# carry4985/ORB_SLAM2_MAP

Hardware: AMD Instinct MI355X
Metric: frames/sec ORB extract+match (640x480, 1000 feat) (higher is better)
Workload: dtype u8; 1 GPU; C2: synthetic 640x480 RGB-D stream, 1000 features, 8 levels, extract + BF-Hamming match of consecutive frames; resident_frame_pool=1024, sequences=1, parallelism=1 sequence per GPU, schedule_name=best, extraction_parts=1

## Files before the change

### include/orbgpu.h

```cpp
#ifndef ORBGPU_H
#define ORBGPU_H

#include <stddef.h>
#include <stdint.h>

#ifdef __cplusplus
extern "C" {
#endif

#define ORBGPU_ABI_VERSION 1
#define ORBGPU_MAX_LEVELS 16

typedef enum {
    ORBGPU_OK = 0,
    ORBGPU_EINVAL = -1,
    ORBGPU_ENOMEM = -2,
    ORBGPU_EHIP = -3,
    ORBGPU_ECAPACITY = -4,
    ORBGPU_ELEVEL = -5
} orbgpu_status;

const char *orbgpu_last_error_string(void);
int orbgpu_abi_version(void);
int orbgpu_device_count(void);
// ... 59 lines not shown
};
int orbgpu_extractor_debug_read(orbgpu_extractor *h, int32_t what, int32_t frame, int32_t level, void *dst,
                                size_t dst_bytes, size_t *n, int32_t *aux);

int orbgpu_extractor_graph_state(const orbgpu_extractor *h, int32_t *state);
int orbgpu_extractor_debug_quadtree_config(const orbgpu_extractor *h, int32_t batch, int32_t *lds_keys, int32_t *threads,
                                           int32_t *lds_bytes);
int orbgpu_extractor_set_profiling(orbgpu_extractor *h, int32_t enable);
int orbgpu_extractor_set_concurrent_blur(orbgpu_extractor *h, int32_t enable);
int orbgpu_extractor_set_fast_early_out(orbgpu_extractor *h, int32_t enable);

int orbgpu_extractor_set_stage_signal(orbgpu_extractor *h, int32_t stage, void *hip_event);
int orbgpu_extractor_stage_count(void);
const char *orbgpu_extractor_stage_name(int32_t i);
int orbgpu_extractor_stage_times(orbgpu_extractor *h, float *ms_out);

typedef struct orbgpu_pipeline orbgpu_pipeline;
int orbgpu_pipeline_create(const orbgpu_extractor_params *params, int32_t parts, orbgpu_pipeline **out);
int orbgpu_pipeline_destroy(orbgpu_pipeline *pl);
int orbgpu_pipeline_parts(const orbgpu_pipeline *pl, int32_t *parts);
int orbgpu_pipeline_part(orbgpu_pipeline *pl, int32_t k, orbgpu_extractor **part);
int orbgpu_pipeline_extract_device(orbgpu_pipeline *pl, const uint8_t *d_gray, int32_t batch, int32_t width,
                                   int32_t height, size_t stride, size_t frame_stride, orbgpu_keypoint *d_kps,
                                   uint8_t *d_desc, int32_t cap, int32_t *d_n_out, void *wait_event, void *done_event);
int orbgpu_pipeline_wait(orbgpu_pipeline *pl, void *hip_stream);


#define ORBGPU_TH_HIGH 100
#define ORBGPU_TH_LOW 50
#define ORBGPU_HISTO_LENGTH 30
#define ORBGPU_GRID_COLS 64
#define ORBGPU_GRID_ROWS 48

int orbgpu_hamming256(const uint8_t *a, const uint8_t *b, int32_t n, int32_t *out, int32_t device_id);

int orbgpu_distinctive_descriptors(int32_t groups, const int32_t *offsets, const uint8_t *desc, int32_t *best_idx,
                                   int32_t device_id);

int orbgpu_match_bf(const uint8_t *desc_a, const float *angle_a, const uint8_t *valid_a, int32_t na,
                    const uint8_t *desc_b, const float *angle_b, int32_t nb, int32_t th_low, float nnratio,
                    int32_t check_orientation, int32_t *match_b, int32_t *nmatches, int32_t device_id);

typedef struct orbgpu_matcher orbgpu_matcher;
int orbgpu_matcher_create(int32_t device_id, int32_t max_pairs, int32_t cap, orbgpu_matcher **out);
int orbgpu_matcher_destroy(orbgpu_matcher *m);
int orbgpu_match_bf_batch_device(orbgpu_matcher *m, int32_t pairs, int32_t cap, const uint8_t *d_desc_a,
                                 const void *d_angle_a, const uint8_t *d_valid_a, const int32_t *d_na,
                                 const uint8_t *d_desc_b, const void *d_angle_b, const int32_t *d_nb,
                                 size_t angle_stride_bytes, int32_t th_low, float nnratio,
                                 int32_t check_orientation, int32_t *d_match_b, int32_t *d_nmatches,
                                 void *hip_stream);
int orbgpu_matcher_last_sweeps(orbgpu_matcher *m, int32_t *sweeps);
int orbgpu_matcher_last_launch(orbgpu_matcher *m, int32_t *nsplit, int32_t *stage_b, int32_t *resolve_threads);

typedef struct {
    int32_t n;
    const float *kp_x, *kp_y;
    const int32_t *kp_octave;
    const float *kp_angle;
    const float *u_right;
    const uint8_t *desc;
    float min_x, max_x, min_y, max_y;
    float grid_inv_w, grid_inv_h;
    const float *scale_factors;
    int32_t nlevels;
    const int32_t *cell_start;
    const int32_t *cell_items;
} orbgpu_frame_view;

int orbgpu_assign_features_to_grid(int32_t n, const float *kp_x, const float *kp_y, float min_x, float min_y,
                                   float grid_inv_w, float grid_inv_h, int32_t *cell_start, int32_t *cell_items);

typedef struct orbgpu_camera {
    float fx, fy, cx, cy;
    float dist[5];
    float mbf;
    float min_x, max_x, min_y, max_y;
} orbgpu_camera;

int orbgpu_undistort_points(int32_t n, const float *xy_in, const orbgpu_camera *cam, float *xy_out, int32_t device_id);

int orbgpu_frame_glue_batch_device(int32_t device_id, int32_t batch, int32_t cap, const orbgpu_keypoint *d_kps,
                                   const int32_t *d_n, const float *d_depth, size_t depth_stride,
                                   size_t depth_frame_stride, const orbgpu_camera *cam, orbgpu_keypoint *d_kps_un,
                                   float *d_u_right, float *d_kp_depth, int32_t *d_cell_start,
                                   int32_t *d_cell_items, void *hip_stream);


int orbgpu_stereo_matches_batch_device(const orbgpu_extractor *left, int32_t left_frame0, const orbgpu_extractor *right,
                                       int32_t right_frame0, int32_t batch, int32_t cap, const orbgpu_keypoint *d_kps_l,
                                       const int32_t *d_n_l, const uint8_t *d_desc_l, const orbgpu_keypoint *d_kps_r,
                                       const int32_t *d_n_r, const uint8_t *d_desc_r, float mbf, float fx,
                                       float *d_u_right, float *d_depth, int32_t *d_n_stereo, void *hip_stream);
int orbgpu_compute_stereo_matches(const orbgpu_extractor *left, const orbgpu_extractor *right, int32_t n_l,
                                  const orbgpu_keypoint *kps_l, const uint8_t *desc_l, int32_t n_r,
                                  const orbgpu_keypoint *kps_r, const uint8_t *desc_r, float mbf, float fx,
                                  float *u_right, float *depth);

typedef struct orbgpu_device_frame_view {
    int32_t cap;
    const int32_t *n;
    const orbgpu_keypoint *kps;
    const uint8_t *desc;
    const float *u_right;
    const int32_t *cell_start;
    const int32_t *cell_items;
// ... 461 lines not shown
```

### orb_slam2_map_amd/csrc/matcher_bf.hip

```cpp
#include "common.h"
#include "matcher_common.h"
#include "staging.h"

#include <algorithm>
#include <climits>
#include <cstdlib>
#include <new>
#include <vector>

namespace orbgpu {

constexpr int BF_TOPK = 4;
constexpr uint32_t BF_KEY_NONE = 0xFFFFFFFFu;

__device__ __forceinline__ uint32_t bf_key(int dist, int j) { return ((uint32_t)dist << 12) | (uint32_t)j; }
__device__ __forceinline__ int bf_key_dist(uint32_t k) { return k == BF_KEY_NONE ? 256 : (int)(k >> 12); }
__device__ __forceinline__ int bf_key_idx(uint32_t k) { return (int)(k & 0xFFFu); }

__device__ __forceinline__ void cswap(uint32_t &a, uint32_t &b)
{
    const uint32_t lo = min(a, b), hi = max(a, b);
    a = lo;
    b = hi;
}

__device__ __forceinline__ void top4_insert(uint32_t t[4], uint32_t k)
{
    if (k < t[3]) {
        t[3] = k;
        cswap(t[2], t[3]);
        cswap(t[1], t[2]);
        cswap(t[0], t[1]);
    }
}

__device__ __forceinline__ void top4_merge(uint32_t t[4], const uint32_t o[4])
{
    uint32_t c0 = min(t[0], o[3]), c1 = min(t[1], o[2]), c2 = min(t[2], o[1]), c3 = min(t[3], o[0]);
    cswap(c0, c2);
    cswap(c1, c3);
    cswap(c0, c1);
    cswap(c2, c3);
    cswap(c1, c2);
    t[0] = c0;
    t[1] = c1;
    t[2] = c2;
    t[3] = c3;
}

constexpr int BF_MIN_SPLIT = 1, BF_MAX_SPLIT = 16;
constexpr size_t BF_RESOLVE_MAX_LDS = 150 * 1024;
constexpr int BF_TILE_STRIDE = 272;
constexpr int BF_TILE_ROWS = 64;
constexpr int BF_TOPK_THREADS = 512;
constexpr int BF_TOPK_ROWS = BF_TOPK_THREADS / 64 * 32;

typedef int v4i __attribute__((ext_vector_type(4)));
typedef int v16i __attribute__((ext_vector_type(16)));

template <uint32_t PM = 0x000001FFu> __device__ __forceinline__ v4i bf_expand16(uint32_t hw)
{
    v4i r;
#pragma unroll
    for (int q = 0; q < 4; q++) {
        const uint32_t n = (hw >> (4 * q)) & 0xFu;
        const uint32_t w01 = __umul24(n, 0x00204081u) & 0x01010101u;
        r[q] = (int)__builtin_amdgcn_perm(0u, PM, w01);
    }
    return r;
}

__device__ __forceinline__ v4i bf_expand16_01(uint32_t hw)
{
    v4i r;
#pragma unroll
    for (int q = 0; q < 4; q++)
        r[q] = (int)(__umul24((hw >> (4 * q)) & 0xFu, 0x00204081u) & 0x01010101u);
    return r;
}

template <bool NODES>
__global__ __launch_bounds__(BF_TOPK_THREADS) void k_bf_topk(int cap, const uint8_t *__restrict__ desc_a,
                                                 const int *__restrict__ na_p, const uint8_t *__restrict__ desc_b,
                                                 const int *__restrict__ nb_p, uint32_t *__restrict__ topk,
                                                 int acc_min, const int *__restrict__ node_a,
                                                 const int *__restrict__ node_b)
{
    __shared__ __align__(16) uint8_t s_tile[2][BF_TILE_ROWS * BF_TILE_STRIDE];
    const int nsplit = gridDim.z;
    const int pair = blockIdx.y;
    const int na = min(na_p[pair], cap);
    const int nb = min(nb_p[pair], cap);
    if ((int)(blockIdx.x * BF_TOPK_ROWS) >= na)
        return;
    const int tid = threadIdx.x, lane = tid & 63, wave = tid >> 6;
    const int r = lane & 31, h = lane >> 5;
    const int i = blockIdx.x * BF_TOPK_ROWS + wave * 32 + r;
    int my_node = 0;
    const int *nodes_b = nullptr;
    if (NODES) {
        my_node = node_a[(size_t)pair * cap + min(i, na - 1)];
        nodes_b = node_b + (size_t)pair * cap;
    }
    v4i fa[8];
    {
        const uint32_t *ga = reinterpret_cast<const uint32_t *>(desc_a + ((size_t)pair * cap + min(i, na - 1)) * 32);
#pragma unroll
        for (int s = 0; s < 8; s++)
            fa[s] = bf_expand16<0x000020E0u>(ga[s] >> (16 * h));
    }
    const int per = (nb + nsplit - 1) / nsplit;
    const int jbeg = (int)blockIdx.z * per, jend = min(nb, jbeg + per);
    const int ntiles = (jend - jbeg + BF_TILE_ROWS - 1) / BF_TILE_ROWS;
    const uint32_t *gb = reinterpret_cast<const uint32_t *>(desc_b + (size_t)pair * cap * 32);
    const int sm = tid >> 3, sw = tid & 7;
    auto fetch = [&](int tile) {
        const int j = min(jbeg + tile * BF_TILE_ROWS + sm, nb - 1);
        return gb[(size_t)j * 8 + sw];
    };
    auto stage = [&](uint32_t d, int buf) {
        v4i *dst = reinterpret_cast<v4i *>(&s_tile[buf][sm * BF_TILE_STRIDE + sw * 32]);
        dst[0] = bf_expand16_01(d);
        dst[1] = bf_expand16_01(d >> 16);
    };
    v16i tag;
    {
        const uint32_t *ga = reinterpret_cast<const uint32_t *>(desc_a + ((size_t)pair * cap + min(i, na - 1)) * 32);
        int pop = 0;
#pragma unroll
        for (int s = 0; s < 8; s++)
            pop += __popc(ga[s]);
        const int sa16 = 16 * (2 * pop - 256);
#pragma unroll
        for (int reg = 0; reg < 16; reg++)
            tag[reg] = (15 - reg) - sa16;
    }
    uint32_t t[4] = {BF_KEY_NONE, BF_KEY_NONE, BF_KEY_NONE, BF_KEY_NONE};
    int lim = acc_min;
    uint32_t d_next = 0;
    if (ntiles > 0)
        stage(fetch(0), 0);
    if (ntiles > 1)
        d_next = fetch(1);
    __syncthreads();
    for (int tile = 0; tile < ntiles; tile++) {
        const uint32_t d_cur = d_next;
        if (tile + 2 < ntiles)
            d_next = fetch(tile + 2);
        if (tile + 1 < ntiles)
            stage(d_cur, (tile + 1) & 1);
        const uint8_t *tb = &s_tile[tile & 1][r * BF_TILE_STRIDE + h * 16];
        v16i acc0 = tag, acc1 = tag;
#pragma unroll
        for (int s = 0; s < 8; s++) {
            const v4i fb0 = *reinterpret_cast<const v4i *>(tb + s * 32);
            const v4i fb1 = *reinterpret_cast<const v4i *>(tb + 32 * BF_TILE_STRIDE + s * 32);
            acc0 = __builtin_amdgcn_mfma_i32_32x32x32_i8(fb0, fa[s], acc0, 0, 0, 0);
            acc1 = __builtin_amdgcn_mfma_i32_32x32x32_i8(fb1, fa[s], acc1, 0, 0, 0);
        }
        const int jlast = jend - 1;
#pragma unroll
        for (int u = 0; u < 2; u++) {
            const v16i &acc = u ? acc1 : acc0;
            int e[16];
#pragma unroll
            for (int reg = 0; reg < 16; reg++)
                e[reg] = acc[reg];
            const int j0 = jbeg + tile * BF_TILE_ROWS + 32 * u + 4 * h;
            for (;;) {
                int m = max(max(e[0], e[1]), e[2]);
#pragma unroll
                for (int reg = 3; reg < 15; reg += 2)
                    m = max(max(m, e[reg]), e[reg + 1]);
                m = max(m, e[15]);
                const bool hit = (m >> 4) >= lim;
                if (!__any(hit))
                    break;
                if (hit) {
                    const int reg = 15 - (m & 15);
                    const int j = j0 + (reg & 3) + 8 * (reg >> 2);
                    if (j <= jlast && (!NODES || nodes_b[j] == my_node)) {
                        top4_insert(t, (uint32_t)(((256 - (m >> 4)) << 11) + j));
                        if (t[3] != BF_KEY_NONE)
                            lim = max(lim, 256 - 2 * (int)(t[3] >> 12));
                    }
#pragma unroll
                    for (int r2 = 0; r2 < 16; r2++)
                        e[r2] = e[r2] == m ? INT_MIN : e[r2];
                }
            }
        }
        __syncthreads();
    }
    {
        uint32_t o[4];
#pragma unroll
        for (int k = 0; k < 4; k++)
            o[k] = __shfl_xor(t[k], 32, 64);
        top4_merge(t, o);
    }
    if (h == 0 && i < na)
        *reinterpret_cast<uint4 *>(topk + (((size_t)pair * cap + i) * nsplit + blockIdx.z) * BF_TOPK) =
            make_uint4(t[0], t[1], t[2], t[3]);
}

__device__ __forceinline__ void bf_full_scan_wave(const uint64_t *__restrict__ ga, const uint64_t *gb, int i, int nb,
                                  const int *claim, int &b1, int &i1, int &b2, const int *__restrict__ nodes_b,
                                  int my_node)
{
    const int lane = threadIdx.x & 63;
    uint64_t a[4] = {ga[(size_t)i * 4], ga[(size_t)i * 4 + 1], ga[(size_t)i * 4 + 2], ga[(size_t)i * 4 + 3]};
    int v1 = 256, vi = INT_MAX, v2 = 256;
    for (int j = lane; j < nb; j += 64) {
        if (claim[j] < i)
            continue;
        if (nodes_b && nodes_b[j] != my_node)
            continue;
        uint64_t b[4] = {gb[(size_t)j * 4], gb[(size_t)j * 4 + 1], gb[(size_t)j * 4 + 2], gb[(size_t)j * 4 + 3]};
        const int d = hamming256(a, b);
        if (d < v1) {
            v2 = v1;
            v1 = d;
            vi = j;
        } else if (d < v2) {
            v2 = d;
        }
    }
#pragma unroll
    for (int off = 32; off > 0; off >>= 1) {
        const int o1 = __shfl_xor(v1, off, 64), oi = __shfl_xor(vi, off, 64), o2 = __shfl_xor(v2, off, 64);
        const bool other_first = (o1 < v1) || (o1 == v1 && oi < vi);
        const int n2 = min(min(v2, o2), max(v1, o1));
        v1 = other_first ? o1 : v1;
        vi = other_first ? oi : vi;
        v2 = n2;
    }
    b1 = v1;
    i1 = vi == INT_MAX ? -1 : vi;
    b2 = v2;
}

__device__ __forceinline__ void bf_load_keys(const uint32_t *__restrict__ tk, int i, int nsplit, uint32_t key[4])
{
    const uint4 k4 = *reinterpret_cast<const uint4 *>(tk + (size_t)i * nsplit * BF_TOPK);
    key[0] = k4.x, key[1] = k4.y, key[2] = k4.z, key[3] = k4.w;
    for (int sp = 1; sp < nsplit; sp++) {
// ... 216 lines not shown
{
    extern __shared__ __align__(16) uint8_t smem[];
    __shared__ unsigned long long s_best;
    uint64_t *sd = reinterpret_cast<uint64_t *>(smem);
    const int g = blockIdx.x, tid = threadIdx.x;
    const int beg = offsets[g], n = offsets[g + 1] - beg;
    if (n <= 0) {
        if (tid == 0)
            best_idx[g] = -1;
        return;
    }
    const uint64_t *gd = reinterpret_cast<const uint64_t *>(desc) + (size_t)beg * 4;
    for (int x = tid; x < n * 4; x += 256)
        sd[x] = gd[x];
    if (tid == 0)
        s_best = ~0ull;
    __syncthreads();
    const int k = (n - 1) >> 1;
    unsigned long long mine = ~0ull;
    for (int i = tid; i < n; i += 256) {
        const uint64_t a[4] = {sd[i * 4], sd[i * 4 + 1], sd[i * 4 + 2], sd[i * 4 + 3]};
        int lo = 0, hi = 256;
        while (lo < hi) {
            const int mid = (lo + hi) >> 1;
            int cnt = 0;
            for (int j = 0; j < n; j++) {
                const uint64_t b[4] = {sd[j * 4], sd[j * 4 + 1], sd[j * 4 + 2], sd[j * 4 + 3]};
                cnt += hamming256(a, b) <= mid ? 1 : 0;
            }
            if (cnt >= k + 1)
                hi = mid;
            else
                lo = mid + 1;
        }
        const unsigned long long key = ((unsigned long long)lo << 32) | (unsigned)i;
        mine = key < mine ? key : mine;
    }
    atomicMin(&s_best, mine);
    __syncthreads();
    if (tid == 0)
        best_idx[g] = (int)(s_best & 0xFFFFFFFFull);
}

}

using namespace orbgpu;

struct orbgpu_matcher {
    int device_id = 0;
    int max_pairs = 0, cap = 0;
    DevBuf d_topk, d_sweeps;
    int last_pairs = 0;
    int resolve_threads = 1024;
    int last_nsplit = 0, last_stage_b = 0;
};

static int matcher_destroy_impl(orbgpu_matcher *m)
{
    if (!m)
        return ORBGPU_OK;
    (void)hipSetDevice(m->device_id);
    (void)hipDeviceSynchronize();
    m->d_topk.release();
    m->d_sweeps.release();
    delete m;
    return ORBGPU_OK;
}

extern "C" {

int orbgpu_matcher_create(int32_t device_id, int32_t max_pairs, int32_t cap, orbgpu_matcher **out)
{
    std::lock_guard<std::mutex> lifecycle(orbgpu::lifecycle_mutex());
    ORBGPU_REQUIRE(out, "null argument");
    ORBGPU_REQUIRE(max_pairs >= 1 && cap >= 1 && cap <= 4096, "max_pairs must be >= 1 and cap in [1,4096]");
    int rc = select_device(device_id);
    if (rc != ORBGPU_OK)
        return rc;
    orbgpu_matcher *m = new (std::nothrow) orbgpu_matcher();
    if (!m) {
        set_error("out of host memory");
        return ORBGPU_ENOMEM;
    }
    m->device_id = device_id;
    m->max_pairs = max_pairs;
    m->cap = cap;
    if (const char *q = getenv("ORBGPU_DEBUG_BF_RESOLVE_THREADS")) {
        const int v = atoi(q);
        if (v == 256 || v == 512 || v == 1024)
            m->resolve_threads = v;
    }
    const size_t P = (size_t)max_pairs;
    if ((rc = m->d_topk.reserve(sizeof(uint32_t) * std::max<size_t>(P * BF_MIN_SPLIT, BF_MAX_SPLIT) * cap * BF_TOPK)) != ORBGPU_OK ||
        (rc = m->d_sweeps.reserve(sizeof(int) * P)) != ORBGPU_OK) {
        matcher_destroy_impl(m);
        return rc;
    }
    hipError_t he = hipFuncSetAttribute(reinterpret_cast<const void *>(k_bf_resolve),
                                 hipFuncAttributeMaxDynamicSharedMemorySize, BF_RESOLVE_MAX_LDS);
    if (he != hipSuccess) {
        set_error("hipFuncSetAttribute: %s", hipGetErrorString(he));
        matcher_destroy_impl(m);
        return ORBGPU_EHIP;
    }
    *out = m;
    return ORBGPU_OK;
}

int orbgpu_matcher_destroy(orbgpu_matcher *m)
{
    std::lock_guard<std::mutex> lifecycle(orbgpu::lifecycle_mutex());
    return matcher_destroy_impl(m);
}

static int match_batch_device(orbgpu_matcher *m, int32_t pairs, int32_t cap, const uint8_t *d_desc_a,
                              const void *d_angle_a, const uint8_t *d_valid_a, const int32_t *d_node_a, const int32_t *d_na,
                              const uint8_t *d_desc_b, const void *d_angle_b, const int32_t *d_node_b, const int32_t *d_nb,
                              size_t angle_stride, int32_t th_low, float nnratio, int32_t check_orientation,
                              int32_t *d_match_b, int32_t *d_nmatches, void *hip_stream)
{
    ORBGPU_REQUIRE(m && d_desc_a && d_desc_b && d_na && d_nb && d_match_b && d_nmatches, "null argument");
    ORBGPU_REQUIRE(pairs >= 1 && pairs <= m->max_pairs && cap >= 1 && cap <= m->cap,
                   "pairs/cap exceed the matcher's capacity (%d pairs, cap %d)", m->max_pairs, m->cap);
    ORBGPU_REQUIRE(!check_orientation || (d_angle_a && d_angle_b && angle_stride >= 4 && angle_stride % 4 == 0),
                   "orientation check needs 4-byte aligned angle arrays");
    int rc = select_device(m->device_id);
    if (rc != ORBGPU_OK)
        return rc;
    hipStream_t st = (hipStream_t)hip_stream;
    uint32_t *topk = m->d_topk.as<uint32_t>();
    int nsplit = BF_MIN_SPLIT;
    while (nsplit < BF_MAX_SPLIT && (size_t)pairs * ((cap + BF_TOPK_ROWS - 1) / BF_TOPK_ROWS) * (BF_TOPK_THREADS / 64) * nsplit < 2048 &&
           (size_t)pairs * nsplit * 2 <= std::max<size_t>((size_t)m->max_pairs * BF_MIN_SPLIT, BF_MAX_SPLIT))
        nsplit *= 2;
    const dim3 grid((cap + BF_TOPK_ROWS - 1) / BF_TOPK_ROWS, pairs, nsplit);
    int dmax = std::min(std::max(th_low, 0), 256);
    while (dmax < 256 && !(nnratio * (float)(dmax + 1) > (float)th_low))
        dmax++;
    if (d_node_a)
        hipLaunchKernelGGL(k_bf_topk<true>, grid, dim3(BF_TOPK_THREADS), 0, st, cap, d_desc_a, d_na, d_desc_b, d_nb, topk,
                           256 - 2 * dmax, d_node_a, d_node_b);
    else
        hipLaunchKernelGGL(k_bf_topk<false>, grid, dim3(BF_TOPK_THREADS), 0, st, cap, d_desc_a, d_na, d_desc_b, d_nb, topk,
                           256 - 2 * dmax, (const int *)nullptr, (const int *)nullptr);
    const int stage_b = (size_t)48 * cap <= BF_RESOLVE_MAX_LDS ? 1 : 0;
    const size_t lds = (size_t)(stage_b ? 48 : 16) * cap;
    hipLaunchKernelGGL(k_bf_resolve, dim3(pairs), dim3(m->resolve_threads), lds, st, cap, d_desc_a, d_valid_a, d_na,
                       d_desc_b, d_nb, topk, th_low, nnratio, reinterpret_cast<const uint8_t *>(d_angle_a),
                       reinterpret_cast<const uint8_t *>(d_angle_b), angle_stride, check_orientation, d_match_b,
                       d_nmatches, m->d_sweeps.as<int>(), stage_b, nsplit, d_node_a, d_node_b);
    ORBGPU_HIP_TRY(hipGetLastError());
    m->last_pairs = pairs;
    m->last_nsplit = nsplit;
    m->last_stage_b = stage_b;
    return ORBGPU_OK;
}

int orbgpu_match_bf_batch_device(orbgpu_matcher *m, int32_t pairs, int32_t cap, const uint8_t *d_desc_a,
                                 const void *d_angle_a, const uint8_t *d_valid_a, const int32_t *d_na,
                                 const uint8_t *d_desc_b, const void *d_angle_b, const int32_t *d_nb,
                                 size_t angle_stride, int32_t th_low, float nnratio, int32_t check_orientation,
                                 int32_t *d_match_b, int32_t *d_nmatches, void *hip_stream)
{
    return match_batch_device(m, pairs, cap, d_desc_a, d_angle_a, d_valid_a, nullptr, d_na, d_desc_b, d_angle_b, nullptr,
                              d_nb, angle_stride, th_low, nnratio, check_orientation, d_match_b, d_nmatches, hip_stream);
}

int orbgpu_search_by_bow_batch_device(orbgpu_matcher *m, int32_t pairs, int32_t cap, const uint8_t *d_desc_a,
                                      const void *d_angle_a, const uint8_t *d_valid_a, const int32_t *d_node_a,
                                      const int32_t *d_na, const uint8_t *d_desc_b, const void *d_angle_b,
                                      const int32_t *d_node_b, const int32_t *d_nb, size_t angle_stride, int32_t th_low,
                                      float nnratio, int32_t check_orientation, int32_t *d_match_b,
                                      int32_t *d_nmatches, void *hip_stream)
{
    ORBGPU_REQUIRE(d_node_a && d_node_b, "null node arrays");
    return match_batch_device(m, pairs, cap, d_desc_a, d_angle_a, d_valid_a, d_node_a, d_na, d_desc_b, d_angle_b, d_node_b,
                              d_nb, angle_stride, th_low, nnratio, check_orientation, d_match_b, d_nmatches, hip_stream);
}

int orbgpu_matcher_last_sweeps(orbgpu_matcher *m, int32_t *sweeps)
{
    ORBGPU_REQUIRE(m && sweeps, "null argument");
    ORBGPU_REQUIRE(m->last_pairs > 0, "no call recorded");
    int rc = select_device(m->device_id);
    if (rc != ORBGPU_OK)
        return rc;
    ORBGPU_HIP_TRY(hipDeviceSynchronize());
    ORBGPU_HIP_TRY(hipMemcpy(sweeps, m->d_sweeps.p, sizeof(int) * m->last_pairs, hipMemcpyDeviceToHost));
    return ORBGPU_OK;
}

int orbgpu_matcher_last_launch(orbgpu_matcher *m, int32_t *nsplit, int32_t *stage_b, int32_t *resolve_threads)
{
    ORBGPU_REQUIRE(m && nsplit && stage_b && resolve_threads, "null argument");
    ORBGPU_REQUIRE(m->last_pairs > 0, "no call recorded");
    *nsplit = m->last_nsplit;
    *stage_b = m->last_stage_b;
    *resolve_threads = m->resolve_threads;
    return ORBGPU_OK;
}

static int match_host(const uint8_t *desc_a, const float *angle_a, const uint8_t *valid_a, const int32_t *node_a,
                      int32_t na, const uint8_t *desc_b, const float *angle_b, const int32_t *node_b, int32_t nb,
                      int32_t th_low, float nnratio, int32_t check_orientation, int32_t *match_b, int32_t *nmatches,
                      int32_t device_id)
{
    ORBGPU_REQUIRE(match_b && nmatches, "null argument");
    ORBGPU_REQUIRE(na >= 0 && nb >= 0 && na <= 4096 && nb <= 4096, "na/nb must be in [0,4096]");
    ORBGPU_REQUIRE((na == 0 || desc_a) && (nb == 0 || desc_b), "null descriptors");
    ORBGPU_REQUIRE(!check_orientation || ((na == 0 || angle_a) && (nb == 0 || angle_b)), "null angles");
    if (na == 0 || nb == 0) {
        int rc = select_device(device_id);
        if (rc != ORBGPU_OK)
            return rc;
        for (int j = 0; j < nb; j++)
            match_b[j] = -1;
        *nmatches = 0;
        return ORBGPU_OK;
    }
    enum { DA, DB, AA, AB, VA, CNT, MB, NM, NDA, NDB, N_BUF };
    struct Ws : Staging<N_BUF> {
        int cap = 0;
        orbgpu_matcher *m = nullptr;
        void drop_matcher()
        {
            if (m)
                orbgpu_matcher_destroy(m);
            m = nullptr;
        }
        ~Ws() { release([this] { drop_matcher(); }); }
    };
    int rc = select_device(device_id);
    if (rc != ORBGPU_OK)
        return rc;
    Ws &ws = per_device_workspace<Ws>(device_id);
    if ((rc = ws.bind(device_id, true)) != ORBGPU_OK)
        return rc;
    const int need = std::max(na, nb);
    if (ws.cap < need) {
        ws.drop_matcher();
        ws.cap = 0;
// ... 153 lines not shown
```

### orb_slam2_map_amd/lib.py

```python
import ctypes as C
import os
import sys

import numpy as np

HERE = os.path.dirname(os.path.abspath(__file__))
LIB_PATH = os.path.join(HERE, "liborbgpu.so")

OK, EINVAL, ENOMEM, EHIP, ECAPACITY, ELEVEL = 0, -1, -2, -3, -4, -5
MAX_LEVELS = 16
GRID_COLS, GRID_ROWS = 64, 48
TH_HIGH, TH_LOW, HISTO_LENGTH = 100, 50, 30

KEYPOINT_DTYPE = np.dtype(
    [("x", "<f4"), ("y", "<f4"), ("size", "<f4"), ("angle", "<f4"), ("response", "<f4"),
     ("octave", "<i4"), ("class_id", "<i4")])
POINT_DTYPE = np.dtype([("x", "<f4"), ("y", "<f4"), ("z", "<f4"), ("rgba", "<u4")])

DBG_PYRAMID_PADDED, DBG_BLURRED_PADDED, DBG_CANDIDATES, DBG_SELECTED, DBG_GRAPH_COUNTS = 0, 1, 2, 3, 4


class OrbGpuError(RuntimeError):
    def __init__(self, status, msg):
        super().__init__("orbgpu status %d: %s" % (status, msg))
# ... 119 lines not shown
        d.update(R12_d=np.array(self.R12_d, np.float64).reshape(3, 3), t12_d=np.array(self.t12_d, np.float64),
                 s12_d=np.float64(self.s12_d), R12=np.array(self.R12, np.float32).reshape(3, 3),
                 t12=np.array(self.t12, np.float32), s12=np.float32(self.s12),
                 T12=np.array(self.T12, np.float32).reshape(4, 4), Scw=np.array(self.Scw, np.float32).reshape(4, 4))
        return d


class Sim3OptProblem(C.Structure):
    _fields_ = [("n1", C.c_int32), ("nlevels", C.c_int32), ("valid", C.c_void_p), ("Xw1", C.c_void_p), ("Xw2", C.c_void_p),
                ("octave1", C.c_void_p), ("octave2", C.c_void_p), ("kp1_xy", C.c_void_p), ("kp2_xy", C.c_void_p),
                ("T1w", C.c_float * 16), ("T2w", C.c_float * 16), ("fx1", C.c_float), ("fy1", C.c_float), ("cx1", C.c_float),
                ("cy1", C.c_float), ("fx2", C.c_float), ("fy2", C.c_float), ("cx2", C.c_float), ("cy2", C.c_float),
                ("inv_level_sigma2", C.c_float * MAX_LEVELS), ("R12", C.c_float * 9), ("t12", C.c_float * 3),
                ("s12", C.c_float), ("th2", C.c_float), ("fix_scale", C.c_int32), ("pad_", C.c_int32),
                ("inlier", C.c_void_p), ("result", C.c_void_p)]


class PnpResult(C.Structure):
    _fields_ = [(k, C.c_int32) for k in ("n", "min_inliers", "max_its", "n_bad_index", "n_bad_set", "accepted", "n_inliers",
                                         "best_inliers", "best_iteration", "iterations", "no_more", "pad_")] + \
               [("Tcw", C.c_float * 16)]

    def as_dict(self):
        d = {k: getattr(self, k) for k, _ in self._fields_[:11]}
        d["Tcw"] = np.array(self.Tcw, np.float32).reshape(4, 4)
        return d


class PnpProblem(C.Structure):
    _fields_ = [("n1", C.c_int32), ("n_hyp", C.c_int32), ("valid", C.c_void_p), ("Xw", C.c_void_p), ("kp", C.c_void_p),
                ("octave", C.c_void_p), ("sets", C.c_void_p), ("fx", C.c_float), ("fy", C.c_float), ("cx", C.c_float),
                ("cy", C.c_float), ("level_sigma2", C.c_float * MAX_LEVELS), ("nlevels", C.c_int32), ("min_set", C.c_int32),
                ("min_inliers", C.c_int32), ("max_iterations", C.c_int32), ("epsilon", C.c_float), ("th2", C.c_float),
                ("probability", C.c_double), ("start_iteration", C.c_int32), ("best_so_far", C.c_int32),
                ("n_iterations", C.c_int32), ("pad_", C.c_int32), ("counts", C.c_void_p), ("Tcw", C.c_void_p),
                ("masks", C.c_void_p), ("refined_mask", C.c_void_p), ("indices", C.c_void_p), ("result", C.c_void_p)]


_LIB = None

ABI_SYMBOLS = [
    "orbgpu_last_error_string", "orbgpu_abi_version", "orbgpu_device_count", "orbgpu_measure_copy_bandwidth",
    "orbgpu_set_trig_mode", "orbgpu_get_trig_mode", "orbgpu_trig_table_info", "orbgpu_trig_host_eval", "orbgpu_trig_eval",
    "orbgpu_extractor_create", "orbgpu_extractor_destroy", "orbgpu_extractor_get_levels",
    "orbgpu_extractor_get_scale_factor", "orbgpu_extractor_get_scale_factors",
    "orbgpu_extractor_get_inv_scale_factors", "orbgpu_extractor_get_sigma2", "orbgpu_extractor_get_inv_sigma2",
    "orbgpu_extractor_get_quotas", "orbgpu_extractor_max_keypoints", "orbgpu_extract", "orbgpu_extract_batch",
    "orbgpu_extract_batch_device", "orbgpu_extractor_get_pyramid_level", "orbgpu_extractor_debug_read",
    "orbgpu_extractor_graph_state", "orbgpu_extractor_debug_quadtree_config", "orbgpu_extractor_set_profiling", "orbgpu_extractor_set_concurrent_blur", "orbgpu_extractor_set_fast_early_out", "orbgpu_extractor_set_stage_signal", "orbgpu_extractor_stage_count", "orbgpu_extractor_stage_name",
    "orbgpu_extractor_stage_times",
    "orbgpu_pipeline_create", "orbgpu_pipeline_destroy", "orbgpu_pipeline_parts", "orbgpu_pipeline_part",
    "orbgpu_pipeline_extract_device", "orbgpu_pipeline_wait",
    "orbgpu_hamming256", "orbgpu_match_bf", "orbgpu_matcher_create", "orbgpu_matcher_destroy",
    "orbgpu_match_bf_batch_device", "orbgpu_matcher_last_sweeps", "orbgpu_matcher_last_launch",
    "orbgpu_assign_features_to_grid",
    "orbgpu_frame_glue_batch_device", "orbgpu_stereo_matches_batch_device", "orbgpu_compute_stereo_matches",
    "orbgpu_undistort_points", "orbgpu_search_local_points_device", "orbgpu_search_local_points_batch_device", "orbgpu_search_by_projection_last_device", "orbgpu_projection_last_sweeps", "orbgpu_distinctive_descriptors", "orbgpu_search_by_projection_sim3",
    "orbgpu_search_by_projection", "orbgpu_search_by_projection_last", "orbgpu_search_by_projection_keyframe",
    "orbgpu_mappoint_table_create", "orbgpu_mappoint_table_destroy", "orbgpu_mappoint_table_rows",
    "orbgpu_mappoint_table_upsert", "orbgpu_mappoint_table_set_bad", "orbgpu_mappoint_table_set_observations",
    "orbgpu_mappoint_table_read", "orbgpu_mappoint_table_last_unknown", "orbgpu_mappoint_table_retain", "orbgpu_frame_create", "orbgpu_frame_destroy", "orbgpu_frame_upload",
    "orbgpu_frame_device_view", "orbgpu_search_local_points_table", "orbgpu_search_by_projection_last_table",
    "orbgpu_pose_optimization", "orbgpu_pose_optimization_device", "orbgpu_pose_optimization_batch_device",
    "orbgpu_pose_optimization_table", "orbgpu_pose_last_spills",
    "orbgpu_sim3_ransac_iterations", "orbgpu_sim3_solve_device", "orbgpu_sim3_solve_batch_device", "orbgpu_sim3_solve",
    "orbgpu_sim3_solve_all",
    "orbgpu_sim3_optimize", "orbgpu_sim3_optimize_device", "orbgpu_sim3_optimize_batch_device",
    "orbgpu_sim3_opt_last_spills",
    "orbgpu_pnp_ransac_parameters", "orbgpu_pnp_solve_device", "orbgpu_pnp_solve_batch_device", "orbgpu_pnp_solve",
    "orbgpu_pnp_solve_all", "orbgpu_pnp_solve_table",
    "orbgpu_keyframe_db_create", "orbgpu_keyframe_db_destroy", "orbgpu_keyframe_db_clear", "orbgpu_keyframe_db_size",
    "orbgpu_keyframe_db_add", "orbgpu_keyframe_db_erase", "orbgpu_keyframe_db_set_covisibles", "orbgpu_keyframe_db_score",
    "orbgpu_keyframe_db_detect_loop", "orbgpu_keyframe_db_detect_reloc", "orbgpu_keyframe_db_last_query",
    "orbgpu_keyframe_db_debug_global_queries",
    "orbgpu_vocabulary_create", "orbgpu_vocabulary_destroy", "orbgpu_vocabulary_size", "orbgpu_bow_transform",
    "orbgpu_bow_transform_batch_device", "orbgpu_search_by_bow", "orbgpu_search_by_bow_batch_device",
    "orbgpu_search_by_bow_keyframes", "orbgpu_search_for_triangulation", "orbgpu_search_for_initialization", "orbgpu_fuse", "orbgpu_fuse_sim3",
    "orbgpu_search_by_sim3",
    "orbgpu_mappoint_record_bytes", "orbgpu_write_mappoint_record", "orbgpu_keyframe_record_bytes",
    "orbgpu_write_keyframe_record", "orbgpu_pcd_binary_header", "orbgpu_write_pcd_binary", "orbgpu_cloud_save_pcd",
    "orbgpu_cloud_create", "orbgpu_cloud_destroy", "orbgpu_cloud_insert", "orbgpu_cloud_insert_device",
    "orbgpu_cloud_clear", "orbgpu_cloud_append_filtered", "orbgpu_cloud_last_path", "orbgpu_cloud_set_profiling", "orbgpu_cloud_last_insert_ms", "orbgpu_cloud_rebuild",
    "orbgpu_cloud_size", "orbgpu_cloud_download", "orbgpu_cloud_last_overflow", "orbgpu_backproject",
    "orbgpu_voxel_filter", "orbgpu_cloud_remove_outliers", "orbgpu_statistical_outlier_removal",
]


def lib():
    global _LIB
    if _LIB is not None:
        return _LIB
    if "torch" not in sys.modules:
        try:
            import torch
        except Exception:
            pass
    if not os.path.exists(LIB_PATH):
        raise OSError("%s is missing: run `python -c 'import __graft_entry__ as g; g.build()'` "
                      "(the HIP extension is the product; there is no CPU fallback)" % LIB_PATH)
    L = C.CDLL(LIB_PATH)
    vp, i32, f32, sz = C.c_void_p, C.c_int32, C.c_float, C.c_size_t
    L.orbgpu_last_error_string.restype = C.c_char_p
    L.orbgpu_extractor_stage_name.restype = C.c_char_p
    L.orbgpu_extractor_stage_name.argtypes = [i32]
    sigs = {
        "orbgpu_extractor_create": [vp, vp],
        "orbgpu_set_trig_mode": [i32],
        "orbgpu_trig_table_info": [vp, vp],
        "orbgpu_extractor_destroy": [vp],
        "orbgpu_extractor_get_levels": [vp, vp],
        "orbgpu_extractor_get_scale_factor": [vp, vp],
        "orbgpu_extractor_get_scale_factors": [vp, vp],
        "orbgpu_extractor_get_inv_scale_factors": [vp, vp],
        "orbgpu_extractor_get_sigma2": [vp, vp],
        "orbgpu_extractor_get_inv_sigma2": [vp, vp],
        "orbgpu_extractor_get_quotas": [vp, vp],
        "orbgpu_extractor_max_keypoints": [vp, i32, i32, vp],
        "orbgpu_extract": [vp, vp, i32, i32, sz, vp, vp, i32, vp],
        "orbgpu_extract_batch": [vp, vp, i32, i32, i32, sz, sz, vp, vp, i32, vp],
        "orbgpu_extract_batch_device": [vp, vp, i32, i32, i32, sz, sz, vp, vp, i32, vp, vp],
        "orbgpu_extractor_get_pyramid_level": [vp, i32, i32, vp, sz, vp, vp],
        "orbgpu_extractor_debug_read": [vp, i32, i32, i32, vp, sz, vp, vp],
        "orbgpu_extractor_set_profiling": [vp, i32],
        "orbgpu_extractor_set_stage_signal": [vp, i32, vp],
        "orbgpu_extractor_stage_times": [vp, vp],
        "orbgpu_pipeline_create": [vp, i32, vp],
        "orbgpu_pipeline_destroy": [vp],
        "orbgpu_pipeline_parts": [vp, vp],
        "orbgpu_pipeline_part": [vp, i32, vp],
        "orbgpu_pipeline_extract_device": [vp, vp, i32, i32, i32, sz, sz, vp, vp, i32, vp, vp, vp],
        "orbgpu_pipeline_wait": [vp, vp],
        "orbgpu_hamming256": [vp, vp, i32, vp, i32],
        "orbgpu_match_bf": [vp, vp, vp, i32, vp, vp, i32, i32, f32, i32, vp, vp, i32],
        "orbgpu_matcher_create": [i32, i32, i32, vp],
        "orbgpu_matcher_destroy": [vp],
        "orbgpu_match_bf_batch_device": [vp, i32, i32, vp, vp, vp, vp, vp, vp, vp, sz, i32, f32, i32, vp, vp, vp],
        "orbgpu_matcher_last_sweeps": [vp, vp],
        "orbgpu_matcher_last_launch": [vp, vp, vp, vp],
        "orbgpu_search_by_bow_batch_device": [vp, i32, i32, vp, vp, vp, vp, vp, vp, vp, vp, vp, sz, i32, f32, i32, vp, vp,
                                              vp],
        "orbgpu_assign_features_to_grid": [i32, vp, vp, f32, f32, f32, f32, vp, vp],
        "orbgpu_frame_glue_batch_device": [i32, i32, i32, vp, vp, vp, sz, sz, vp, vp, vp, vp, vp, vp, vp],
        "orbgpu_stereo_matches_batch_device": [vp, i32, vp, i32, i32, i32, vp, vp, vp, vp, vp, vp, f32, f32, vp, vp, vp,
                                               vp],
        "orbgpu_compute_stereo_matches": [vp, vp, i32, vp, vp, i32, vp, vp, f32, f32, vp, vp],
        "orbgpu_undistort_points": [i32, vp, vp, vp, i32],
        "orbgpu_search_local_points_device": [vp, vp, vp, f32, f32, f32, f32, f32, f32, f32, f32, f32, vp, vp, vp, i32, vp],
        "orbgpu_projection_last_sweeps": [vp, vp],
        "orbgpu_distinctive_descriptors": [i32, vp, vp, vp, i32],
        "orbgpu_search_by_projection_sim3": [vp, vp, f32, f32, f32, f32, f32, vp, i32, vp, vp, i32],
        "orbgpu_search_by_projection": [vp, vp, f32, f32, vp, vp, i32],
        "orbgpu_search_by_projection_last": [vp, vp, f32, f32, f32, f32, f32, f32, vp, f32, i32, i32, vp, vp, i32],
        "orbgpu_search_by_projection_keyframe": [vp, vp, f32, f32, f32, f32, f32, vp, f32, i32, i32, vp, vp, i32],
        "orbgpu_cloud_create": [C.c_double, i32, vp],
        "orbgpu_cloud_destroy": [vp],
        "orbgpu_cloud_insert": [vp, vp, sz, vp, sz, i32, i32, f32, f32, f32, f32, vp],
        "orbgpu_cloud_insert_device": [vp, vp, sz, vp, sz, i32, i32, f32, f32, f32, f32, vp],
        "orbgpu_cloud_last_path": [vp, vp],
        "orbgpu_cloud_set_profiling": [vp, i32],
        "orbgpu_cloud_last_insert_ms": [vp, vp],
        "orbgpu_cloud_rebuild": [vp, i32, vp, sz, vp, sz, i32, i32, f32, f32, f32, f32, vp],
        "orbgpu_cloud_size": [vp, vp],
        "orbgpu_cloud_download": [vp, vp, C.c_int64, vp],
        "orbgpu_cloud_last_overflow": [vp, vp],
        "orbgpu_backproject": [vp, sz, vp, sz, i32, i32, f32, f32, f32, f32, vp, vp, C.c_int64, vp, i32],
        "orbgpu_voxel_filter": [vp, C.c_int64, C.c_double, vp, C.c_int64, vp, vp, i32],
        "orbgpu_cloud_remove_outliers": [vp, i32, C.c_double, vp],
        "orbgpu_statistical_outlier_removal": [vp, C.c_int64, i32, C.c_double, vp, C.c_int64, vp, vp, i32],
        "orbgpu_keyframe_db_create": [i32, i32, i32, i32, vp],
        "orbgpu_keyframe_db_destroy": [vp],
        "orbgpu_keyframe_db_clear": [vp],
        "orbgpu_keyframe_db_size": [vp, vp],
        "orbgpu_keyframe_db_add": [vp, C.c_int64, i32, vp, vp],
        "orbgpu_keyframe_db_erase": [vp, i32, vp, vp],
        "orbgpu_keyframe_db_set_covisibles": [vp, C.c_int64, i32, vp],
        "orbgpu_keyframe_db_score": [vp, i32, vp, vp, i32, vp, vp],
        "orbgpu_keyframe_db_detect_loop": [vp, i32, vp, vp, i32, vp, f32, i32, vp, vp],
        "orbgpu_keyframe_db_detect_reloc": [vp, i32, vp, vp, i32, vp, vp],
        "orbgpu_keyframe_db_last_query": [vp, i32, vp, vp, vp, vp, vp, vp, vp],
        "orbgpu_keyframe_db_debug_global_queries": [vp, vp],
    }
    for name, args in sigs.items():
        fn = getattr(L, name, None)
        if fn is not None:
            fn.argtypes = args
            fn.restype = C.c_int
    _LIB = L
    return L


def check(status):
# ... 1093 lines not shown
    d2 = np.ascontiguousarray(desc2, np.uint8).reshape(-1, 32)
    a1, a2 = np.ascontiguousarray(angle1, np.float32), np.ascontiguousarray(angle2, np.float32)
    v1 = None if valid1 is None else np.ascontiguousarray(valid1, np.uint8)
    v2 = None if valid2 is None else np.ascontiguousarray(valid2, np.uint8)
    nd1, nd2 = np.ascontiguousarray(node1, np.int32), np.ascontiguousarray(node2, np.int32)
    out = np.full(max(len(d1), 1), -1, np.int32)
    n = C.c_int32()
    L = lib()
    L.orbgpu_search_by_bow_keyframes.argtypes = [C.c_void_p] * 4 + [C.c_int32] + [C.c_void_p] * 4 + [C.c_int32, C.c_float,
                                                                                                   C.c_int32, C.c_void_p,
                                                                                                   C.c_void_p, C.c_int32]
    check(L.orbgpu_search_by_bow_keyframes(_p(d1), _p(a1), _p(v1), _p(nd1), len(d1), _p(d2), _p(a2), _p(v2), _p(nd2),
                                           len(d2), nnratio, int(check_ori), _p(out), C.byref(n), device_id))
    return n.value, out[:len(d1)]


class BatchMatcher:

    def __init__(self, max_pairs, cap, device_id=0):
        self.L = lib()
        h = C.c_void_p()
        check(self.L.orbgpu_matcher_create(device_id, max_pairs, cap, C.byref(h)))
        self.h, self.max_pairs, self.cap = h, max_pairs, cap

    def close(self):
        if getattr(self, "h", None):
            self.L.orbgpu_matcher_destroy(self.h)
            self.h = None

    __del__ = close

    def match(self, pairs, cap, d_desc_a, d_angle_a, d_valid_a, d_na, d_desc_b, d_angle_b, d_nb, angle_stride,
              th_low, nnratio, check_ori, d_match_b, d_nmatches, stream=0):
        check(self.L.orbgpu_match_bf_batch_device(self.h, pairs, cap, d_desc_a, d_angle_a, d_valid_a, d_na, d_desc_b,
                                                  d_angle_b, d_nb, angle_stride, th_low, nnratio, int(check_ori),
                                                  d_match_b, d_nmatches, stream))

    def search_by_bow(self, pairs, cap, d_desc_a, d_angle_a, d_valid_a, d_node_a, d_na, d_desc_b, d_angle_b, d_node_b,
                      d_nb, angle_stride, th_low, nnratio, check_ori, d_match_b, d_nmatches, stream=0):
        check(self.L.orbgpu_search_by_bow_batch_device(self.h, pairs, cap, d_desc_a, d_angle_a, d_valid_a, d_node_a, d_na,
                                                       d_desc_b, d_angle_b, d_node_b, d_nb, angle_stride, th_low, nnratio,
                                                       int(check_ori), d_match_b, d_nmatches, stream))

    def last_sweeps(self, pairs):
        out = np.zeros(pairs, np.int32)
        check(self.L.orbgpu_matcher_last_sweeps(self.h, _p(out)))
        return out

    def last_launch(self):
        v = [C.c_int32() for _ in range(3)]
        check(self.L.orbgpu_matcher_last_launch(self.h, *[C.byref(x) for x in v]))
        return dict(nsplit=v[0].value, stage_b=v[1].value, resolve_threads=v[2].value)


def keyframe_record(kf_id, timestamp, Tcw, keys, desc, mappoint_index):
    L = lib()
    L.orbgpu_keyframe_record_bytes.restype = C.c_size_t
    L.orbgpu_keyframe_record_bytes.argtypes = [C.c_int32]
    L.orbgpu_write_keyframe_record.argtypes = [C.c_uint64, C.c_double, C.c_void_p, C.c_int32, C.c_void_p, C.c_void_p,
                                               C.c_void_p, C.c_void_p, C.c_size_t, C.c_void_p]
    keys = np.ascontiguousarray(keys, KEYPOINT_DTYPE)
    desc = np.ascontiguousarray(desc, np.uint8).reshape(-1, 32)
    idx = np.ascontiguousarray(mappoint_index, np.uint64)
    T = np.ascontiguousarray(Tcw, np.float32)
    n = len(keys)
    out = np.zeros(L.orbgpu_keyframe_record_bytes(n), np.uint8)
    w = C.c_size_t()
    check(L.orbgpu_write_keyframe_record(kf_id, timestamp, _p(T), n, _p(keys) if n else None, _p(desc) if n else None,
                                         _p(idx) if n else None, _p(out), len(out), C.byref(w)))
    return out[:w.value].tobytes()


def mappoint_record(mp_id, world_pos):
    L = lib()
    L.orbgpu_write_mappoint_record.argtypes = [C.c_uint64, C.c_void_p, C.c_void_p, C.c_size_t, C.c_void_p]
    p = np.ascontiguousarray(world_pos, np.float32)
    out = np.zeros(20, np.uint8)
    w = C.c_size_t()
    check(L.orbgpu_write_mappoint_record(mp_id, _p(p), _p(out), 20, C.byref(w)))
    return out[:w.value].tobytes()


def pcd_binary_header(n):
    L = lib()
    L.orbgpu_pcd_binary_header.argtypes = [C.c_int64, C.c_char_p, C.c_size_t, C.c_void_p]
    buf = C.create_string_buffer(512)
    w = C.c_size_t()
    check(L.orbgpu_pcd_binary_header(n, buf, 512, C.byref(w)))
    return buf.raw[:w.value]


TF_IDF, TF, IDF, BINARY = 0, 1, 2, 3
L1_NORM, L2_NORM, CHI_SQUARE, KL, BHATTACHARYYA, DOT_PRODUCT = range(6)


class ORBVocabulary:

    def __init__(self, k, L, parent, is_leaf, desc, weight, weighting=TF_IDF, scoring=L1_NORM, device_id=0):
        self.L_ = lib()
        self.parent = np.ascontiguousarray(parent, np.int32)
        self.is_leaf = np.ascontiguousarray(is_leaf, np.uint8)
        self.desc = np.ascontiguousarray(desc, np.uint8).reshape(-1, 32)
        self.weight = np.ascontiguousarray(weight, np.float64)
        self.k, self.L, self.device_id = k, L, device_id
        h = C.c_void_p()
        fn = self.L_.orbgpu_vocabulary_create
# ... 278 lines not shown
```

Measured before the change: 303,400 frames/s.

## Replace per-tile max-extraction loop with branch-free LDS candidate list and batched compaction

The BF top-k kernel no longer runs a data-dependent loop that repeatedly extracts the maximum accumulator per tile. Every MFMA result is now encoded and written to a per-thread LDS list, advancing the slot pointer only for entries above the current threshold. The list is compacted into the top-4 set only when any lane nears capacity, and once more at the end. The next tile's first fragments are also prefetched after a moved barrier. This adds about 36KB of dynamic LDS per block, which may reduce occupancy, plus debug entry points to read the top-k keys and list capacity.

```diff
diff --git a/include/orbgpu.h b/include/orbgpu.h
--- a/include/orbgpu.h
+++ b/include/orbgpu.h
@@ -135,6 +135,8 @@
                                  void *hip_stream);
 int orbgpu_matcher_last_sweeps(orbgpu_matcher *m, int32_t *sweeps);
 int orbgpu_matcher_last_launch(orbgpu_matcher *m, int32_t *nsplit, int32_t *stage_b, int32_t *resolve_threads);
+int orbgpu_matcher_last_topk(orbgpu_matcher *m, uint32_t *keys, size_t n_keys);
+int orbgpu_matcher_list_cap(orbgpu_matcher *m, int32_t *list_cap, int32_t *list_cap_min);
 
 typedef struct {
     int32_t n;
diff --git a/orb_slam2_map_amd/csrc/matcher_bf.hip b/orb_slam2_map_amd/csrc/matcher_bf.hip
--- a/orb_slam2_map_amd/csrc/matcher_bf.hip
+++ b/orb_slam2_map_amd/csrc/matcher_bf.hip
@@ -54,6 +54,9 @@
 constexpr int BF_TILE_ROWS = 64;
 constexpr int BF_TOPK_THREADS = 512;
 constexpr int BF_TOPK_ROWS = BF_TOPK_THREADS / 64 * 32;
+constexpr int BF_LIST_MIN = 16;
+constexpr int BF_LIST_CAP = 18;
+constexpr size_t BF_LIST_LDS = (size_t)BF_LIST_CAP * BF_TOPK_THREADS * sizeof(uint32_t);
 
 typedef int v4i __attribute__((ext_vector_type(4)));
 typedef int v16i __attribute__((ext_vector_type(16)));
@@ -83,10 +86,11 @@
 __global__ __launch_bounds__(BF_TOPK_THREADS) void k_bf_topk(int cap, const uint8_t *__restrict__ desc_a,
                                                  const int *__restrict__ na_p, const uint8_t *__restrict__ desc_b,
                                                  const int *__restrict__ nb_p, uint32_t *__restrict__ topk,
-                                                 int acc_min, const int *__restrict__ node_a,
+                                                 int acc_min, int list_cap, const int *__restrict__ node_a,
                                                  const int *__restrict__ node_b)
 {
     __shared__ __align__(16) uint8_t s_tile[2][BF_TILE_ROWS * BF_TILE_STRIDE];
+    extern __shared__ __align__(16) uint32_t s_list[];
     const int nsplit = gridDim.z;
     const int pair = blockIdx.y;
     const int na = min(na_p[pair], cap);
@@ -137,12 +141,36 @@
     }
     uint32_t t[4] = {BF_KEY_NONE, BF_KEY_NONE, BF_KEY_NONE, BF_KEY_NONE};
     int lim = acc_min;
+    constexpr uint32_t SLOT = BF_TOPK_THREADS * sizeof(uint32_t);
+    static_assert(SLOT == 1u << 11, "the append below advances by a shift of 11");
+    uint32_t *pos = s_list + tid;
+    const uint32_t *const pos_full = s_list + tid + BF_TOPK_THREADS * (list_cap - BF_LIST_MIN);
+    const int jlast = jend - 1;
+    auto key_of = [&](uint32_t en, bool listed) {
+        const int a = (int)(en >> 13) + lim * 16, reg = 15 - (a & 15);
+        const int j = (int)(en & 0x1FFFu) + (reg & 3) + 8 * (reg >> 2);
+        const bool live = listed && j <= jlast && (!NODES || nodes_b[min(j, jlast)] == my_node);
+        return live ? (uint32_t)(((256 - (a >> 4)) << 11) + j) : BF_KEY_NONE;
+    };
+    auto compact = [&]() {
+        static_assert(BF_LIST_CAP % 2 == 0 && BF_LIST_MIN % 2 == 0, "the second entry of a trip must be inside the list");
+        for (const uint32_t *p = s_list + tid; __any(p < pos); p += 2 * BF_TOPK_THREADS) {
+            const uint32_t k0 = key_of(p[0], p < pos), k1 = key_of(p[BF_TOPK_THREADS], p + BF_TOPK_THREADS < pos);
+            top4_insert(t, k0);
+            top4_insert(t, k1);
+        }
+        pos = s_list + tid;
+        if (t[3] != BF_KEY_NONE)
+            lim = max(lim, 256 - 2 * (int)(t[3] >> 12));
+    };
     uint32_t d_next = 0;
     if (ntiles > 0)
         stage(fetch(0), 0);
     if (ntiles > 1)
         d_next = fetch(1);
     __syncthreads();
+    const uint8_t *const tb0 = &s_tile[0][r * BF_TILE_STRIDE + h * 16];
+    v4i nf0 = *reinterpret_cast<const v4i *>(tb0), nf1 = *reinterpret_cast<const v4i *>(tb0 + 32 * BF_TILE_STRIDE);
     for (int tile = 0; tile < ntiles; tile++) {
         const uint32_t d_cur = d_next;
         if (tile + 2 < ntiles)
@@ -153,45 +181,37 @@
         v16i acc0 = tag, acc1 = tag;
 #pragma unroll
         for (int s = 0; s < 8; s++) {
-            const v4i fb0 = *reinterpret_cast<const v4i *>(tb + s * 32);
-            const v4i fb1 = *reinterpret_cast<const v4i *>(tb + 32 * BF_TILE_STRIDE + s * 32);
+            const v4i fb0 = s ? *reinterpret_cast<const v4i *>(tb + s * 32) : nf0;
+            const v4i fb1 = s ? *reinterpret_cast<const v4i *>(tb + 32 * BF_TILE_STRIDE + s * 32) : nf1;
             acc0 = __builtin_amdgcn_mfma_i32_32x32x32_i8(fb0, fa[s], acc0, 0, 0, 0);
             acc1 = __builtin_amdgcn_mfma_i32_32x32x32_i8(fb1, fa[s], acc1, 0, 0, 0);
         }
-        const int jlast = jend - 1;
+        __builtin_amdgcn_sched_barrier(0);
+        __syncthreads();
+        {
+            const uint8_t *nb0 = &s_tile[(tile + 1) & 1][r * BF_TILE_STRIDE + h * 16];
+            nf0 = *reinterpret_cast<const v4i *>(nb0);
+            nf1 = *reinterpret_cast<const v4i *>(nb0 + 32 * BF_TILE_STRIDE);
+        }
 #pragma unroll
         for (int u = 0; u < 2; u++) {
             const v16i &acc = u ? acc1 : acc0;
-            int e[16];
-#pragma unroll
-            for (int reg = 0; reg < 16; reg++)
-                e[reg] = acc[reg];
-            const int j0 = jbeg + tile * BF_TILE_ROWS + 32 * u + 4 * h;
-            for (;;) {
-                int m = max(max(e[0], e[1]), e[2]);
-#pragma unroll
-                for (int reg = 3; reg < 15; reg += 2)
-                    m = max(max(m, e[reg]), e[reg + 1]);
-                m = max(m, e[15]);
-                const bool hit = (m >> 4) >= lim;
-                if (!__any(hit))
-                    break;
-                if (hit) {
-                    const int reg = 15 - (m & 15);
-                    const int j = j0 + (reg & 3) + 8 * (reg >> 2);
-                    if (j <= jlast && (!NODES || nodes_b[j] == my_node)) {
-                        top4_insert(t, (uint32_t)(((256 - (m >> 4)) << 11) + j));
-                        if (t[3] != BF_KEY_NONE)
-                            lim = max(lim, 256 - 2 * (int)(t[3] >> 12));
-                    }
-#pragma unroll
-                    for (int r2 = 0; r2 < 16; r2++)
-                        e[r2] = e[r2] == m ? INT_MIN : e[r2];
-                }
+            const int jb = jbeg + tile * BF_TILE_ROWS + 32 * u + 4 * h - lim * (16 << 13);
+            typedef __attribute__((address_space(3))) uint32_t lds_u32;
+            uint32_t q = (uint32_t)(uintptr_t)(lds_u32 *)pos;
+#pragma unroll
+            for (int reg = 0; reg < 16; reg++) {
+                const int en = acc[reg] * (1 << 13) + jb;
+                *(lds_u32 *)(uintptr_t)(q + reg * SLOT) = (uint32_t)en;
+                const int m = en >> 31;
+                asm("v_lshl_add_u32 %0, %1, 11, %0" : "+v"(q) : "v"(m));
             }
-        }
-        __syncthreads();
-    }
+            pos += (int)(q - (uint32_t)(uintptr_t)(lds_u32 *)pos) / 4 + 16 * BF_TOPK_THREADS;
+            if (__any(pos > pos_full))
+                compact();
+        }
+    }
+    compact();
     {
         uint32_t o[4];
 #pragma unroll
@@ -514,7 +534,9 @@
     DevBuf d_topk, d_sweeps;
     int last_pairs = 0;
     int resolve_threads = 1024;
+    int list_cap = BF_LIST_CAP;
     int last_nsplit = 0, last_stage_b = 0;
+    int last_cap = 0;
 };
 
 static int matcher_destroy_impl(orbgpu_matcher *m)
@@ -552,6 +574,11 @@
         if (v == 256 || v == 512 || v == 1024)
             m->resolve_threads = v;
     }
+    if (const char *q = getenv("ORBGPU_DEBUG_BF_LIST_CAP")) {
+        const int v = atoi(q);
+        if (v >= BF_LIST_MIN && v < BF_LIST_CAP)
+            m->list_cap = v;
+    }
     const size_t P = (size_t)max_pairs;
     if ((rc = m->d_topk.reserve(sizeof(uint32_t) * std::max<size_t>(P * BF_MIN_SPLIT, BF_MAX_SPLIT) * cap * BF_TOPK)) != ORBGPU_OK ||
         (rc = m->d_sweeps.reserve(sizeof(int) * P)) != ORBGPU_OK) {
@@ -560,6 +587,12 @@
     }
     hipError_t he = hipFuncSetAttribute(reinterpret_cast<const void *>(k_bf_resolve),
                                  hipFuncAttributeMaxDynamicSharedMemorySize, BF_RESOLVE_MAX_LDS);
+    if (he == hipSuccess)
+        he = hipFuncSetAttribute(reinterpret_cast<const void *>(k_bf_topk<false>), hipFuncAttributeMaxDynamicSharedMemorySize,
+                                 BF_LIST_LDS);
+    if (he == hipSuccess)
+        he = hipFuncSetAttribute(reinterpret_cast<const void *>(k_bf_topk<true>), hipFuncAttributeMaxDynamicSharedMemorySize,
+                                 BF_LIST_LDS);
     if (he != hipSuccess) {
         set_error("hipFuncSetAttribute: %s", hipGetErrorString(he));
         matcher_destroy_impl(m);
@@ -600,11 +633,11 @@
     while (dmax < 256 && !(nnratio * (float)(dmax + 1) > (float)th_low))
         dmax++;
     if (d_node_a)
-        hipLaunchKernelGGL(k_bf_topk<true>, grid, dim3(BF_TOPK_THREADS), 0, st, cap, d_desc_a, d_na, d_desc_b, d_nb, topk,
-                           256 - 2 * dmax, d_node_a, d_node_b);
+        hipLaunchKernelGGL(k_bf_topk<true>, grid, dim3(BF_TOPK_THREADS), BF_LIST_LDS, st, cap, d_desc_a, d_na, d_desc_b, d_nb,
+                           topk, 256 - 2 * dmax, m->list_cap, d_node_a, d_node_b);
     else
-        hipLaunchKernelGGL(k_bf_topk<false>, grid, dim3(BF_TOPK_THREADS), 0, st, cap, d_desc_a, d_na, d_desc_b, d_nb, topk,
-                           256 - 2 * dmax, (const int *)nullptr, (const int *)nullptr);
+        hipLaunchKernelGGL(k_bf_topk<false>, grid, dim3(BF_TOPK_THREADS), BF_LIST_LDS, st, cap, d_desc_a, d_na, d_desc_b, d_nb,
+                           topk, 256 - 2 * dmax, m->list_cap, (const int *)nullptr, (const int *)nullptr);
     const int stage_b = (size_t)48 * cap <= BF_RESOLVE_MAX_LDS ? 1 : 0;
     const size_t lds = (size_t)(stage_b ? 48 : 16) * cap;
     hipLaunchKernelGGL(k_bf_resolve, dim3(pairs), dim3(m->resolve_threads), lds, st, cap, d_desc_a, d_valid_a, d_na,
@@ -615,6 +648,7 @@
     m->last_pairs = pairs;
     m->last_nsplit = nsplit;
     m->last_stage_b = stage_b;
+    m->last_cap = cap;
     return ORBGPU_OK;
 }
 
@@ -649,6 +683,28 @@
         return rc;
     ORBGPU_HIP_TRY(hipDeviceSynchronize());
     ORBGPU_HIP_TRY(hipMemcpy(sweeps, m->d_sweeps.p, sizeof(int) * m->last_pairs, hipMemcpyDeviceToHost));
+    return ORBGPU_OK;
+}
+
+int orbgpu_matcher_last_topk(orbgpu_matcher *m, uint32_t *keys, size_t n_keys)
+{
+    ORBGPU_REQUIRE(m && keys, "null argument");
+    ORBGPU_REQUIRE(m->last_pairs > 0, "no call recorded");
+    const size_t n = (size_t)m->last_pairs * m->last_cap * m->last_nsplit * BF_TOPK;
+    ORBGPU_REQUIRE(n_keys == n, "the last call left %zu keys, not %zu", n, n_keys);
+    int rc = select_device(m->device_id);
+    if (rc != ORBGPU_OK)
+        return rc;
+    ORBGPU_HIP_TRY(hipDeviceSynchronize());
+    ORBGPU_HIP_TRY(hipMemcpy(keys, m->d_topk.p, sizeof(uint32_t) * n, hipMemcpyDeviceToHost));
+    return ORBGPU_OK;
+}
+
+int orbgpu_matcher_list_cap(orbgpu_matcher *m, int32_t *list_cap, int32_t *list_cap_min)
+{
+    ORBGPU_REQUIRE(m && list_cap && list_cap_min, "null argument");
+    *list_cap = m->list_cap;
+    *list_cap_min = BF_LIST_MIN;
     return ORBGPU_OK;
 }
 
diff --git a/orb_slam2_map_amd/lib.py b/orb_slam2_map_amd/lib.py
--- a/orb_slam2_map_amd/lib.py
+++ b/orb_slam2_map_amd/lib.py
@@ -195,7 +195,8 @@
     "orbgpu_pipeline_create", "orbgpu_pipeline_destroy", "orbgpu_pipeline_parts", "orbgpu_pipeline_part",
     "orbgpu_pipeline_extract_device", "orbgpu_pipeline_wait",
     "orbgpu_hamming256", "orbgpu_match_bf", "orbgpu_matcher_create", "orbgpu_matcher_destroy",
-    "orbgpu_match_bf_batch_device", "orbgpu_matcher_last_sweeps", "orbgpu_matcher_last_launch",
+    "orbgpu_match_bf_batch_device", "orbgpu_matcher_last_sweeps", "orbgpu_matcher_last_launch", "orbgpu_matcher_last_topk",
+    "orbgpu_matcher_list_cap",
     "orbgpu_assign_features_to_grid",
     "orbgpu_frame_glue_batch_device", "orbgpu_stereo_matches_batch_device", "orbgpu_compute_stereo_matches",
     "orbgpu_undistort_points", "orbgpu_search_local_points_device", "orbgpu_search_local_points_batch_device", "orbgpu_search_by_projection_last_device", "orbgpu_projection_last_sweeps", "orbgpu_distinctive_descriptors", "orbgpu_search_by_projection_sim3",
@@ -280,6 +281,8 @@
         "orbgpu_match_bf_batch_device": [vp, i32, i32, vp, vp, vp, vp, vp, vp, vp, sz, i32, f32, i32, vp, vp, vp],
         "orbgpu_matcher_last_sweeps": [vp, vp],
         "orbgpu_matcher_last_launch": [vp, vp, vp, vp],
+        "orbgpu_matcher_last_topk": [vp, vp, sz],
+        "orbgpu_matcher_list_cap": [vp, vp, vp],
         "orbgpu_search_by_bow_batch_device": [vp, i32, i32, vp, vp, vp, vp, vp, vp, vp, vp, vp, sz, i32, f32, i32, vp, vp,
                                               vp],
         "orbgpu_assign_features_to_grid": [i32, vp, vp, f32, f32, f32, f32, vp, vp],
@@ -1479,6 +1482,16 @@
         check(self.L.orbgpu_matcher_last_launch(self.h, *[C.byref(x) for x in v]))
         return dict(nsplit=v[0].value, stage_b=v[1].value, resolve_threads=v[2].value)
 
+    def list_cap(self):
+        v = [C.c_int32(), C.c_int32()]
+        check(self.L.orbgpu_matcher_list_cap(self.h, C.byref(v[0]), C.byref(v[1])))
+        return v[0].value, v[1].value
+
+    def last_topk(self, pairs, cap):
+        out = np.zeros((pairs, cap, self.last_launch()["nsplit"], 4), np.uint32)
+        check(self.L.orbgpu_matcher_last_topk(self.h, _p(out), out.size))
+        return out
+
 
 def keyframe_record(kf_id, timestamp, Tcw, keys, desc, mappoint_index):
     L = lib()
```

Result: no change. 302,400 frames/s (-0.3%).
